# zjhellofss/KuiperLLama

Hardware: NVIDIA H100
Metric: decode_tokens_per_s (higher is better)
Workload: dtype f32

## Files before the change

kuiperllama_b200/csrc/megakernel.cu:

```cuda
#include <cooperative_groups.h>
#include <cuda_bf16.h>
#include <cuda_runtime.h>

#include <cfloat>
#include <cstdint>
#include <algorithm>
#include <cstdio>
#include <cstdlib>
#include <string>
#include <vector>

#include "../../include/kllm_b200.h"
#include "kllm_device.cuh"
#include "kllm_host.h"
#include "kv_fp8.cuh"
#include "megakernel.h"

namespace kllm {
namespace mega {

#define KLLM_MBAR_HINT_NS 20000u
#define KLLM_PHASE_CALL __forceinline__
#define KLLM_STAGE_CALL __noinline__
constexpr int kMaxStages = 16;
constexpr int kConsumerWarps = 8;
constexpr int kConsumerThreads = kConsumerWarps * 32;
constexpr int kSoftmaxThreads = 256;
constexpr int kNormThreads = 128;
constexpr long long kSpinLimit = 120000000000LL;

__device__ __forceinline__ uint32_t smem_u32(const void* p) {
  return static_cast<uint32_t>(__cvta_generic_to_shared(p));
}
__device__ __forceinline__ void mbar_init(uint64_t* b, int count) {
  asm volatile("mbarrier.init.shared::cta.b64 [%0], %1;" ::"r"(smem_u32(b)), "r"(count));
}
__device__ __forceinline__ void mbar_expect_tx(uint64_t* b, uint32_t bytes) {
  asm volatile("mbarrier.arrive.expect_tx.shared::cta.b64 _, [%0], %1;" ::"r"(smem_u32(b)),
               "r"(bytes)
               : "memory");
}
__device__ __forceinline__ void mbar_arrive(uint64_t* b) {
  asm volatile("mbarrier.arrive.shared::cta.b64 _, [%0];" ::"r"(smem_u32(b)) : "memory");
}
__device__ __forceinline__ void mbar_wait(uint64_t* b, uint32_t parity) {
  asm volatile(
      "{\n .reg .pred p;\n WAIT_%=:\n"
      " mbarrier.try_wait.parity.shared::cta.b64 p, [%0], %1, %2;\n"
      " @p bra DONE_%=;\n bra WAIT_%=;\n DONE_%=:\n}" ::"r"(smem_u32(b)),
// ... 130 lines not shown
}

struct Pipe {
  int slot;
  uint32_t parity;
  __device__ __forceinline__ void advance(int stages) {
    if (++slot == stages) {
      slot = 0;
      parity ^= 1u;
    }
  }
};

__shared__ uint64_t g_full_bar[kMaxStages];
__shared__ uint64_t g_empty_bar[kMaxStages];
__shared__ float g_s_warp[kConsumerWarps];
__shared__ float g_s_argv[kConsumerWarps];
__shared__ int g_s_argi[kConsumerWarps];
__shared__ float g_s_bcast;
__shared__ volatile int g_stop;
__shared__ volatile unsigned g_prod_end;
__shared__ Phase g_ph_cons;
__shared__ Phase g_ph_prod;
extern __shared__ __align__(128) unsigned char smem[];
struct Carry {
  Pipe pipe;
  float best_v;
  int best_i;
};

__device__ __forceinline__ void grid_barrier(unsigned* counter, unsigned& target, unsigned grid) {
  consumer_sync();
  target += grid;
  if (threadIdx.x == 0) {
    red_release_add(counter, 1u);
    while (static_cast<int>(ld_acquire_u32(counter) - target) < 0) {
    }
  }
  consumer_sync();
}

struct RowRef {
  int seg;
  int row;
};
__device__ __forceinline__ RowRef resolve_row(const Phase& ph, int unit, int sub) {
// ... 83 lines not shown
    for (int r = 0; r < NR; ++r)
#pragma unroll
      for (int j = 0; j < 4; ++j) wv[r][j] = lds_pack<F>(wp[r] + 32 * PB * j);
#pragma unroll
    for (int j = 0; j < 4; ++j)
#pragma unroll
      for (int r = 0; r < NR; ++r) acc[r][j] = __fadd_rn(dot4_ref(xv[j], wv[r][j]), acc[r][j]);
    xp += 2048;
#pragma unroll
    for (int r = 0; r < NR; ++r) wp[r] += 128 * PB;
  }
  if (full < n_packs) {
#pragma unroll
    for (int j = 0; j < 4; ++j) {
      if (full + 32 * j + lane < n_packs) {
        const float4 xv = lds_f4(xp + 512 * j);
#pragma unroll
        for (int r = 0; r < NR; ++r) acc[r][j] = __fadd_rn(dot4_ref(xv, lds_pack<F>(wp[r] + 32 * PB * j)), acc[r][j]);
      }
    }
  }
}

template <int NR>
__device__ __forceinline__ void accum_w8_g64(const uint32_t (&w)[NR], const uint32_t (&sc)[NR], uint32_t x,
                                             int M, int lane, float (&acc)[NR][4]) {
  const int chunks = M >> 7;
  const bool tail = (chunks << 7) + (lane << 2) < M;
  const int total = chunks + (tail ? 1 : 0);
  if (total == 0) return;
  uint32_t xp = x + lane * 16;
  uint32_t wp[NR], sp[NR];
#pragma unroll
  for (int r = 0; r < NR; ++r) {
    wp[r] = w[r] + lane * 4;
    sp[r] = sc[r] + (lane >> 4) * 4;
  }
  float4 xv = lds_f4(xp);
  uint32_t packed[NR];
  float s[NR];
#pragma unroll
  for (int r = 0; r < NR; ++r) {
    packed[r] = lds_u32(wp[r]);
    s[r] = lds_f32(sp[r]);
  }
#pragma unroll 2
// ... 133 lines not shown
      uint32_t* o1 = reinterpret_cast<uint32_t*>(gb + ((1u + odd) & 3u) * 64);
      uint32_t* o2 = reinterpret_cast<uint32_t*>(gb + ((2u + odd) & 3u) * 64);
#pragma unroll
      for (int j = 0; j < 4; ++j) {
        const float e[4] = {v[j].x, v[j].y, v[j].z, v[j].w};
        uint32_t p0 = 0, p1 = 0, p2 = 0;
#pragma unroll
        for (int b = 0; b < 4; ++b) {
          const int qv = __float2int_rn(e[b] * inv);
          const int a0 = ((qv + 128) & 255) - 128;
          const int q1 = (qv - a0) >> 8;
          const int a1 = ((q1 + 128) & 255) - 128;
          const int a2 = (q1 - a1) >> 8;
          p0 |= static_cast<uint32_t>(a0 & 255) << (8 * b);
          p1 |= static_cast<uint32_t>(a1 & 255) << (8 * b);
          p2 |= static_cast<uint32_t>(a2 & 255) << (8 * b);
        }
        o0[j] = p0, o1[j] = p1, o2[j] = p2;
      }
      if (q == 0) *reinterpret_cast<float*>(gb + ((3u + odd) & 3u) * 64) = step;
    }
  }
  consumer_sync();
}

struct Rows4 {
  uint32_t a[4];
};
template <int NR, WeightFormat F>
__device__ __forceinline__ float4 dot_rows(Rows4 rows, Rows4 scales, uint32_t x, int M, int group_size,
                                           int group_shift, int lane, bool fast = false) {
  float acc[NR][4];
#pragma unroll
  for (int r = 0; r < NR; ++r)
#pragma unroll
    for (int j = 0; j < 4; ++j) acc[r][j] = 0.f;
  float d[4] = {0.f, 0.f, 0.f, 0.f};
  uint32_t w[NR], sc[NR];
#pragma unroll
  for (int r = 0; r < NR; ++r) {
    w[r] = rows.a[r];
    sc[r] = scales.a[r];
  }
  if constexpr (F == WeightFormat::kInt8) {
    if (fast) {
      float a1[NR];
// ... 1148 lines not shown
  return id;
}

template <WeightFormat F, int KV, bool LP, bool PROF>
__device__ __forceinline__ void megakernel_body(const Params& P) {
  uint64_t* full_bar = g_full_bar;
  uint64_t* empty_bar = g_empty_bar;
  Phase& s_phase_cons = g_ph_cons;
  Phase& s_phase_prod = g_ph_prod;

  float* xres = reinterpret_cast<float*>(smem + P.xbuf_bytes);
  unsigned char* stages = smem + P.xbuf_bytes + P.xres_bytes;
  const int S = P.num_stages;
  const int tid = threadIdx.x;
  const int lane = tid & 31;
  const int warp = tid >> 5;
  const bool is_producer = warp == kConsumerWarps;
  const int cta = blockIdx.x;
  const int G = gridDim.x;

  if (tid == 0) {
    g_stop = 0;
    g_prod_end = 0u;
    for (int s = 0; s < S; ++s) {
      mbar_init(&full_bar[s], 1);
      mbar_init(&empty_bar[s], kConsumerWarps);
    }
    asm volatile("fence.mbarrier_init.release.cluster;" ::: "memory");
  }
  __syncthreads();

  Pipe pipe{0, 0u};
  constexpr int wbytes = weight_bytes(F);

  if (is_producer) {
    const uint64_t policy = policy_evict_first();
    const uint64_t policy_kv = policy_evict_last();
    int ppos = P.state->pos;
    unsigned long long* pstamp = nullptr;
    auto claim_slot = [&](uint32_t bytes) -> unsigned char* {
      const long long pw0 = PROF ? clock64() : 0;
      if (mbar_wait_or_stop(&empty_bar[pipe.slot], pipe.parity ^ 1u, &g_stop)) return nullptr;
      if constexpr (PROF) {
        if (pstamp && lane == 0) {
          atomicAdd(pstamp + 11, static_cast<unsigned long long>(clock64() - pw0));
          atomicAdd(pstamp + 12, 1ull);
        }
      }
      if (lane == 0) mbar_expect_tx(&full_bar[pipe.slot], bytes);
      __syncwarp();
      return stages + static_cast<size_t>(pipe.slot) * P.stage_bytes;
    };
    for (int tok = 0; tok < P.n_tokens; ++tok, ++ppos) {
      const int n_run = tok < P.skip_cls_tokens ? P.n_phases - P.n_cls_phases : P.n_phases;
      for (int pi = 0; pi < n_run; ++pi) {
        if constexpr (PROF)
          pstamp = (P.prof != nullptr && tok == P.prof_token)
                       ? P.prof + (static_cast<size_t>(cta) * P.n_phases + pi) * kProfStamps
                       : nullptr;
        {
          const uint32_t* src = reinterpret_cast<const uint32_t*>(P.phases + pi);
          uint32_t* dst = reinterpret_cast<uint32_t*>(&s_phase_prod);
          __syncwarp();
          for (int i = lane; i < static_cast<int>(sizeof(Phase) / 4); i += 32) dst[i] = __ldg(src + i);
          __syncwarp();
        }
        const Phase& ph = s_phase_prod;
        if (ph.kind == kPhaseGather) continue;
        if (ph.kind != kPhaseGemv) {
          const int SP = P.attn_split;
          if (cta >= P.head_num * SP || ppos == 0) continue;
// ... 57 lines not shown
            }
          }
          if (ph.kind != kPhaseAttention) {
            const int dv = hs / SP, T = P.attn_tile_v;
            const float* vbase = P.value_cache + head_block + static_cast<size_t>(split) * P.seq_len * dv;
            const int n_tiles = attn_tiles(ppos, T);
            for (int j = 0; j < n_tiles; ++j) {
              const int t0 = j * T;
              const int nt = min(T, ppos - t0);
              unsigned char* dst = claim_slot(static_cast<uint32_t>(nt) * dv * 4);
              if (dst == nullptr) goto producer_done;
              if (lane == 0)
                bulk_g2s(dst, vbase + static_cast<size_t>(t0) * dv, static_cast<uint32_t>(nt) * dv * 4,
                         &full_bar[pipe.slot], policy_kv);
              pipe.advance(S);
            }
          }
          continue;
        }
        const int u0 = static_cast<int>(static_cast<long long>(cta) * ph.units / G);
        const int u1 = static_cast<int>(static_cast<long long>(cta + 1) * ph.units / G);
        const int rpu = ph.swiglu ? 2 : 1;
        const int row_bytes = ph.in_dim * wbytes;
        if (ph.chunks_per_row == 1) {
          const int ups = ph.rows_per_stage / rpu;
          for (int u = u0; u < u1; u += ups) {
            const int n = min(ups, u1 - u);
            const int nrows = n * rpu;
            unsigned char* dst = claim_slot(static_cast<uint32_t>(nrows) * (row_bytes + ph.scale_row_bytes));
            if (dst == nullptr) goto producer_done;
            const RowRef rr = lane < nrows ? stage_row(ph, u, n, lane) : RowRef{-1, -1};
            const int len = run_length(rr, lane, nrows);
            if (len > 0) {
              const long long e = static_cast<long long>(rr.row) * ph.in_dim;
              const unsigned char* src = static_cast<const unsigned char*>(ph.seg[rr.seg].w) + e * wbytes;
              bulk_g2s(dst + static_cast<size_t>(lane) * row_bytes, src, static_cast<uint32_t>(len) * row_bytes,
                       &full_bar[pipe.slot], policy);
              if (ph.scale_row_bytes) {
                const long long g0 = ph.group_shift >= 0 ? (e >> ph.group_shift) : (e / ph.group_size);
                bulk_g2s(dst + ph.scale_off + static_cast<size_t>(lane) * ph.scale_row_bytes,
                         ph.seg[rr.seg].scales + g0, static_cast<uint32_t>(len) * ph.scale_row_bytes,
                         &full_bar[pipe.slot], policy);
              }
            }
            pipe.advance(S);
          }
        } else {
          for (int u = u0; u < u1; ++u) {
            const RowRef rr = resolve_row(ph, u, 0);
            const unsigned char* src = static_cast<const unsigned char*>(ph.seg[rr.seg].w) +
                                       static_cast<long long>(rr.row) * row_bytes;
            for (int c = 0; c < ph.chunks_per_row; ++c) {
              const int e0 = c * ph.chunk_elems;
              const int ne = min(ph.chunk_elems, ph.in_dim - e0);
              unsigned char* dst = claim_slot(static_cast<uint32_t>(ne) * wbytes);
              if (dst == nullptr) goto producer_done;
              if (lane == 0)
                bulk_g2s(dst, src + static_cast<size_t>(e0) * wbytes, static_cast<uint32_t>(ne) * wbytes,
                         &full_bar[pipe.slot], policy);
              pipe.advance(S);
            }
          }
        }
      }
    }
  producer_done:
    if (lane == 0) g_prod_end = 1u + ((static_cast<unsigned>(pipe.slot) << 1) | pipe.parity);
    return;
  }

  unsigned bar_target = P.barrier_base;
  int token = P.state->token;
  int pos = P.state->pos;
  record_fed(P, pos, token);
  if (static_cast<unsigned>(token) >= static_cast<unsigned>(P.vocab_size)) token = 0;
  int step = P.state->step;
  float4* xres4 = reinterpret_cast<float4*>(xres);
  constexpr int kPhaseWords = static_cast<int>(sizeof(Phase) / 4);
  static_assert(kPhaseWords <= kConsumerThreads, "phase copy: one word per consumer thread");
  uint32_t next_phase_word = tid < kPhaseWords ? __ldg(reinterpret_cast<const uint32_t*>(P.phases) + tid) : 0u;

  for (int tok = 0; tok < P.n_tokens; ++tok) {
    const float* emb_row = P.tok_emb + static_cast<size_t>(token) * P.dim;
    ArgBest best{0.f, -1};
    const float4* e4 = reinterpret_cast<const float4*>(emb_row);
    for (int i = tid; i < (P.dim >> 2); i += kConsumerThreads) xres4[i] = __ldg(e4 + i);

    const bool prof_on = PROF && P.prof != nullptr && tok == P.prof_token && tid == 0;
    auto hand_tag = [&](int hand) {
      return P.hand_base + static_cast<unsigned>(tok * P.hands_per_token + hand) + 1u;
// ... 64 lines not shown
    step += 1;
    if (cta == 0 && tid == 0 && (tok == P.n_tokens - 1 || stop)) {
      P.state->token = token;
      P.state->pos = pos;
      P.state->step = step;
      P.state->next = next;
    }
    if (stop) {
      if (tid == 0) g_stop = 1;
      unsigned end;
      while ((end = g_prod_end) == 0u) {
      }
      const Pipe last{static_cast<int>((end - 1u) >> 1), (end - 1u) & 1u};
      while (pipe.slot != last.slot || pipe.parity != last.parity) {
        mbar_wait(&full_bar[pipe.slot], pipe.parity);
        pipe.advance(S);
      }
      return;
    }
  }
}

template <WeightFormat F, int KV, bool LP, bool PROF>
__global__ void __launch_bounds__(kConsumerThreads + 32, 1) decode_megakernel(const __grid_constant__ Params P) {
  megakernel_body<F, KV, LP, PROF>(P);
}

}

using mega::Params;
using mega::Phase;

namespace {
template <typename K>
const void* fn(K* kernel) {
  return reinterpret_cast<const void*>(kernel);
}
struct Kernels {
  const void *plain, *prof, *lp;
};
template <WeightFormat F, int KV>
Kernels kernels_for() {
  using mega::decode_megakernel;
  const void* prof = nullptr;
  if constexpr (F != WeightFormat::kBf16 && KV == KLLM_KV_F32) prof = fn(decode_megakernel<F, KV, false, true>);
  return Kernels{fn(decode_megakernel<F, KV, false, false>), prof, fn(decode_megakernel<F, KV, true, false>)};
}
template <WeightFormat F>
Kernels kernels_for(int kv) {
  switch (kv) {
    case KLLM_KV_BF16: return kernels_for<F, KLLM_KV_BF16>();
    case KLLM_KV_FP8: return kernels_for<F, KLLM_KV_FP8>();
    default: return kernels_for<F, KLLM_KV_F32>();
  }
}
Kernels kernels_for(WeightFormat f, int kv) {
  switch (f) {
    case WeightFormat::kInt8: return kernels_for<WeightFormat::kInt8>(kv);
    case WeightFormat::kBf16: return kernels_for<WeightFormat::kBf16>(kv);
    default: return kernels_for<WeightFormat::kF32>(kv);
  }
}
constexpr int kThreads = mega::kConsumerThreads + 32;
constexpr int kW16StageBytes = 32 * 1024;
constexpr int kW16FastStageBytes = 24 * 1024;
}

int MegaEngine::init(const DecoderModel& dm, const MegaModel& m, cudaStream_t stream) {
  int dev = 0;
  if (cudaGetDevice(&dev) != cudaSuccess) return KLLM_E_NODEVICE;
  int sms = 0, coop = 0, max_smem = 0;
  KLLM_TRY(cudaDeviceGetAttribute(&sms, cudaDevAttrMultiProcessorCount, dev));
  KLLM_TRY(cudaDeviceGetAttribute(&coop, cudaDevAttrCooperativeLaunch, dev));
  KLLM_TRY(cudaDeviceGetAttribute(&max_smem, cudaDevAttrMaxSharedMemoryPerBlockOptin, dev));
  if (!coop) return KLLM_E_UNSUPPORTED;

  const int dim = dm.dim, hid = dm.hidden_dim, hs = dm.head_size, kvd = dm.kv_dim, q_rows = dm.q_rows;
  const bool int8 = dm.format == WeightFormat::kInt8;
  const bool w16 = dm.format == WeightFormat::kBf16;
  const int wb = weight_bytes(dm.format);
  const int grid = std::min(sms, std::min(dim, hid));
  if (grid < dm.head_num) return KLLM_E_UNSUPPORTED;
  if ((dim & 3) || (hid & 3) || (q_rows & 3) || (hs & 3) || hs > 128) return KLLM_E_UNSUPPORTED;
  if (int8 && ((dim & 15) || (hid & 15) || (q_rows & 15) || (dm.group_size & 3))) return KLLM_E_UNSUPPORTED;
  if (w16 && ((dim & 7) || (hid & 7) || (q_rows & 7))) return KLLM_E_UNSUPPORTED;
  if ((hs * 4) % 16 != 0) return KLLM_E_UNSUPPORTED;
  if (int8) {
    const int dims[3] = {dim, hid, q_rows};
    for (int d : dims)
      if (d % dm.group_size != 0 || ((d / dm.group_size) * 4) % 16 != 0) return KLLM_E_UNSUPPORTED;
  }
  int fast = m.numerics == 1 ? 1 : 0;
  if (const char* e = getenv("KLLM_MODE")) fast = std::string(e) == "fast" ? 1 : 0;
  const int kv = m.kv_cache;
  if (kv != KLLM_KV_F32 && kv != KLLM_KV_BF16 && kv != KLLM_KV_FP8) return KLLM_E_INVALID;
  const int kv_esz = prefill::kv_elem_bytes(kv);
  if (kv != KLLM_KV_F32 && (!fast || m.tp_world > 1 || hs % (64 / kv_esz) != 0)) return KLLM_E_UNSUPPORTED;
  if (kv == KLLM_KV_FP8 && m.kv_scales == nullptr) return KLLM_E_INVALID;
  const Kernels ks = kernels_for(dm.format, kv);

  const int W = m.tp_world > 1 ? m.tp_world : 1;
  if (W != 1 && W != 2 && W != 4 && W != 8) return KLLM_E_UNSUPPORTED;

  const int max_in = std::max(std::max(dim, hid), q_rows);
  int xbuf = max_in * 4;
  const int attn_ws = 2 * hs * 4;
  xbuf = std::max(xbuf, attn_ws);
  const bool small_stages = fast && kv == KLLM_KV_F32 && !w16 && 2 * dim * 4 <= 16 * 1024;
  int stage_bytes = int8 ? 27 * 1024 : w16 ? (fast ? kW16FastStageBytes : kW16StageBytes) : small_stages ? 16 * 1024
                                                                                                : 32 * 1024;
  if (const char* e = getenv("KLLM_STAGE_BYTES")) stage_bytes = atoi(e);
  stage_bytes = (stage_bytes + 127) & ~127;
  const int attn_tile = std::min(stage_bytes / (hs * kv_esz), mega::kConsumerThreads) & ~31;
  if (attn_tile < 32) return KLLM_E_UNSUPPORTED;
  if (fast) {
    if (hs & 15) return KLLM_E_UNSUPPORTED;
    xbuf = std::max(xbuf, (2 * hs + mega::kConsumerWarps * (hs + 2)) * 4);
  }
  xbuf = std::max(xbuf, sampling::kDrawScratchBase + 64 * 8);
  xbuf = std::max(xbuf, sampling::logprob_scratch_bytes(mega::kConsumerThreads));
  xbuf = (xbuf + 127) & ~127;
  const int xres = (dim * 4 + 127) & ~127;
  const int budget = max_smem - xbuf - xres - 3584;
  int stages = budget / stage_bytes;
  if (stages > mega::kMaxStages) stages = mega::kMaxStages;
  if (stages < 2) return KLLM_E_UNSUPPORTED;
  if (dm.seq_len & 3) return KLLM_E_UNSUPPORTED;
  int split = 1;
  while (split * 2 <= 8 && dm.head_num * split * 2 <= grid && (hs / (split * 2)) % 4 == 0 && hs % (split * 2) == 0)
    split *= 2;
  int split_cap = split;
  if (hs < 128) split = 1;
  if (fast) {
    split = 1;
// ... 35 lines not shown
      const int chunk_max = (stage_bytes / wb) & ~511;
      p.chunks_per_row = (p.in_dim + chunk_max - 1) / chunk_max;
      int ce = (p.in_dim + p.chunks_per_row - 1) / p.chunks_per_row;
      ce = (ce + 511) & ~511;
      p.chunk_elems = ce;
      p.chunks_per_row = (p.in_dim + ce - 1) / ce;
      p.rows_per_stage = 1;
      p.scale_off = 0;
    }
    return 0;
  };
  Phase qkv{}, wo{}, ffn{}, w2{}, cls{};
  qkv.in_dim = dim, wo.in_dim = q_rows, ffn.in_dim = dim, ffn.swiglu = 1, w2.in_dim = hid, cls.in_dim = dim;
  for (Phase* p : {&qkv, &wo, &ffn, &w2, &cls})
    if (int rc = plan(*p)) return rc;
  const int V = dm.vocab_size;
  const bool shard = W > 1 && V % W == 0 && m.tp_stride >= V / W;
  const int cls_rows = shard ? V / W : V;

  for (const void* k : {ks.plain, ks.prof, ks.lp})
    if (k != nullptr)
      if (int rc = smem_opt_in(k, smem_bytes)) return rc;
  int occ_lp = 0;
  KLLM_TRY(cudaOccupancyMaxActiveBlocksPerMultiprocessor(&occ_lp, ks.lp, kThreads, smem_bytes));
  if (occ_lp < 1) return KLLM_E_UNSUPPORTED;
  int occ = 0;
  KLLM_TRY(cudaOccupancyMaxActiveBlocksPerMultiprocessor(&occ, ks.plain, kThreads, smem_bytes));
  if (occ < 1) return KLLM_E_UNSUPPORTED;

  const int n_phases = dm.layer_num * ((fast || split == 1) ? 5 : 6) + (shard ? 2 : 1);
  size_t bytes = 0;
  auto part = [&bytes](size_t n) {
    const size_t off = bytes;
    bytes += (n + 255) & ~static_cast<size_t>(255);
    return off;
  };
  using u64 = unsigned long long;
  const size_t hand_off = part(sizeof(u64) * (2 * q_rows + 2 * kvd + hid));
  const size_t scores_off = part(sizeof(u64) * dm.head_num * dm.seq_len);
  const size_t probs_off = part(fast || split == 1 ? 0 : sizeof(float) * dm.head_num * split * dm.seq_len);
  const size_t tagged_off = part(W == 1 ? sizeof(u64) * 2 * dim : 0);
  const size_t phases_off = part(sizeof(Phase) * n_phases);
  const size_t barrier_off = part(128);
  const size_t arg_val_off = part(sizeof(float) * grid), arg_idx_off = part(sizeof(int) * grid);
  const size_t lp_off = part(static_cast<size_t>(grid) * (sizeof(float2) + 8 * sampling::kMaxTopLogprobs));
  KLLM_TRY(cudaMalloc(&scratch_, bytes));
  unsigned char* const s = static_cast<unsigned char*>(scratch_);
  u64 *t_q = reinterpret_cast<u64*>(s + hand_off), *t_k = t_q + q_rows, *t_v = t_k + kvd, *t_attn = t_v + kvd,
      *t_h = t_attn + q_rows;

  std::vector<Phase> ph;
  int hands = 0;
  int exch = 0;
  auto input_is_x = [&](Phase& p) {
    if (exch == 0) return;
    p.tp_in = 1;
    p.exch = exch - 1;
  };

  auto seg = [](const Matrix& w, float* out, int rows, int head_major = 0, unsigned long long* tag_out = nullptr) {
    return mega::Seg{w.w, w.scales, w.bias, out, 0, rows, head_major, tag_out};
  };
  for (int l = 0; l < dm.layer_num; ++l) {
    const LayerWeights& lw = dm.layers[l];
    const size_t layer_off = static_cast<size_t>(l) * dm.seq_len * kvd;
    {
      Phase p = qkv;
      p.kind = mega::kPhaseGemv;
      p.n_seg = 3;
      input_is_x(p);
      p.norm_w = lw.attn_norm;
      p.norm_eps = dm.eps;
      p.seg[0] = seg(lw.q, nullptr, q_rows, 0, t_q);
      p.seg[1] = seg(lw.k, nullptr, kvd, 0, t_k);
      float* vrows = reinterpret_cast<float*>(reinterpret_cast<unsigned char*>(m.value_cache) + layer_off * kv_esz);
      p.seg[2] = seg(lw.v, vrows, kvd, 1, t_v);
      p.layer = l;
      p.units = q_rows + 2 * kvd;
      p.hand_out = hands;
      ph.push_back(p);
    }
    if (fast || split == 1) {
      Phase p{};
      p.kind = fast ? mega::kPhaseAttnFlash : mega::kPhaseAttnFused;
      p.layer = l;
      p.tq = t_q, p.tk = t_k, p.tv = t_v, p.ta = t_attn;
      p.hand_in = hands++;
      p.hand_out = hands;
      ph.push_back(p);
    } else {
      int qkv_hand = 0;
      {
        Phase p{};
        p.kind = mega::kPhaseAttention;
        p.layer = l;
        p.tq = t_q, p.tk = t_k, p.tv = t_v;
        p.hand_in = hands++;
        qkv_hand = p.hand_in;
        p.hand_out = hands;
        ph.push_back(p);
      }
      {
        Phase p{};
        p.kind = mega::kPhaseAttnPV;
        p.layer = l;
        p.hand_in = hands++;
        p.tv = t_v, p.ta = t_attn;
        p.hand_aux = qkv_hand;
        p.hand_out = hands;
        ph.push_back(p);
      }
    }
    {
      Phase p = wo;
      p.kind = mega::kPhaseGemv;
      p.n_seg = 1;
      p.tag_in = t_attn;
      p.hand_in = hands++;
      p.seg[0] = seg(lw.o, nullptr, dim);
      p.units = dim;
      p.tp_out = 1;
      p.exch_out = exch++;
      ph.push_back(p);
    }
    {
      Phase p = ffn;
      p.kind = mega::kPhaseGemv;
      p.n_seg = 2;
      input_is_x(p);
      p.norm_w = lw.ffn_norm;
      p.norm_eps = dm.eps;
      p.seg[0] = seg(lw.w1, nullptr, hid, 0, t_h);
      p.seg[1] = seg(lw.w3, nullptr, hid);
      p.units = hid;
      p.hand_out = hands;
      ph.push_back(p);
    }
    {
      Phase p = w2;
      p.kind = mega::kPhaseGemv;
      p.n_seg = 1;
      p.tag_in = t_h;
      p.hand_in = hands++;
      p.seg[0] = seg(lw.w2, nullptr, dim);
      p.units = dim;
      p.tp_out = 1;
      p.exch_out = exch++;
      ph.push_back(p);
    }
  }
  {
    Phase p = cls;
    p.kind = mega::kPhaseGemv;
    p.n_seg = 1;
    input_is_x(p);
    p.norm_w = dm.final_norm;
    p.norm_eps = dm.eps;
    p.cls = 1;
    if (shard) {
      p.seg[0] = seg(dm.rows_from(dm.cls, static_cast<size_t>(m.tp_rank) * cls_rows, dim), nullptr, cls_rows);
      p.units = cls_rows;
      p.tp_out = 1;
      p.exch_out = exch++;
      ph.push_back(p);
      Phase g{};
      g.kind = mega::kPhaseGather;
      g.cls = 1;
      g.argmax = 1;
      g.units = V;
      g.in_dim = cls_rows;
      g.exch = p.exch_out;
      g.seg[0].out = m.logits;
      ph.push_back(g);
    } else {
      p.seg[0] = seg(dm.cls, m.logits, V);
      p.units = V;
      p.argmax = 1;
      ph.push_back(p);
    }
  }

  KLLM_TRY(cudaMemsetAsync(s, 0, bytes, stream));
  KLLM_TRY(cudaMemcpyAsync(s + phases_off, ph.data(), sizeof(Phase) * n_phases, cudaMemcpyHostToDevice, stream));
  KLLM_TRY(cudaStreamSynchronize(stream));

  Params P{};
  P.phases = reinterpret_cast<const Phase*>(s + phases_off);
  P.n_phases = n_phases;
  P.n_cls_phases = shard ? 2 : 1;
  P.int8_fast = (int8 && fast) ? 1 : 0;
  P.num_stages = stages;
  P.stage_bytes = stage_bytes;
  P.xbuf_bytes = xbuf;
  P.xres_bytes = xres;
  P.attn_tile = attn_tile;
  P.attn_tile_v = attn_tile_v;
  P.attn_split = split;
  P.attn_vsplit = vsplit;
  P.scores = reinterpret_cast<u64*>(s + scores_off);
  P.group_size = dm.group_size;
  P.dim = dm.dim;
  P.vocab_size = dm.vocab_size;
  P.head_num = dm.head_num;
  P.head_size = dm.head_size;
  P.kv_dim = dm.kv_dim;
  P.kv_mul = dm.kv_mul;
  P.seq_len = dm.seq_len;
  P.flavour = dm.flavour;
  P.tok_emb = dm.tok_emb;
  P.score = m.score;
  P.probs = reinterpret_cast<float*>(s + probs_off);
  P.key_cache = m.key_cache;
  P.value_cache = m.value_cache;
  P.sin_cache = m.sin_cache;
  P.cos_cache = m.cos_cache;
  P.state = m.state;
  P.out_tokens = m.out_tokens;
// ... 10 lines not shown
  P.arg_idx = reinterpret_cast<int*>(s + arg_idx_off);
  P.sampling = m.sampling;
  P.logits = m.logits;
  P.hist = m.hist;
  P.penalized = m.penalized;
  P.prof_token = -1;
  for (int i = 0; i < mega::kMaxStopIds; ++i) P.stop_ids[i] = -1;
  P.lp_part = reinterpret_cast<float2*>(s + lp_off);
  P.lp_cand_v = reinterpret_cast<float*>(P.lp_part + grid);
  P.lp_cand_i = reinterpret_cast<int*>(P.lp_cand_v + static_cast<size_t>(grid) * sampling::kMaxTopLogprobs);
  P.lp_rec = m.lp_rec;
  if (kv == KLLM_KV_FP8) {
    const size_t n = static_cast<size_t>(dm.layer_num) * dm.kv_head_num;
    P.kv_scale_k = m.kv_scales, P.kv_scale_v = m.kv_scales + n;
    P.kv_inv_k = m.kv_scales + 2 * n, P.kv_inv_v = m.kv_scales + 3 * n;
  }
  base_ = P;
  stream_ = stream;
  grid_ = grid;
  fast_ = fast;
  cls_rows_ = cls_rows;
  kernel_ = ks.plain, kernel_prof_ = ks.prof, kernel_lp_ = ks.lp;
  smem_bytes_ = smem_bytes;
  ready_ = true;
  return 0;
}

int MegaEngine::destroy() {
  const cudaError_t e = cudaFree(scratch_);
  scratch_ = nullptr;
  ready_ = false;
  return static_cast<int>(e);
}

Params MegaEngine::params(const DrawSettings& cfg, int n_tokens) const {
  Params P = base_;
  P.n_tokens = n_tokens;
  P.penalty = cfg.penalty;
  P.lp_top_n = cfg.lp_top_n;
  P.barrier_base = barrier_base_;
  P.tp_seq_base = tp_seq_base_;
  P.hand_base = hand_base_;
  return P;
}

int MegaEngine::launch(const Params& P) {
  void* args[] = {const_cast<Params*>(&P)};
  const void* k = P.prof != nullptr ? kernel_prof_ : P.lp_top_n >= 0 ? kernel_lp_ : kernel_;
  if (k == nullptr) return KLLM_E_UNSUPPORTED;
  KLLM_TRY(cudaLaunchCooperativeKernel(const_cast<void*>(k), dim3(grid_), dim3(kThreads), args, smem_bytes_, stream_));
  count_launch();
  return 0;
}

void MegaEngine::account(int n_tokens) {
  tp_seq_base_ += static_cast<unsigned>(n_tokens) * static_cast<unsigned>(base_.exch_per_token);
  hand_base_ += static_cast<unsigned>(n_tokens) * static_cast<unsigned>(base_.hands_per_token);
  barrier_base_ += static_cast<unsigned>(n_tokens) * static_cast<unsigned>(grid_);
}

int MegaEngine::run(const DrawSettings& cfg, int n_tokens, const int32_t* teacher_dev, unsigned long long* prof_dev,
                    int prof_token, int skip_cls_tokens, int lp_target) {
  if (!ready_) return KLLM_E_STATE;
  Params P = params(cfg, n_tokens);
  P.teacher = teacher_dev;
  P.prof = prof_dev;
  P.prof_token = prof_token;
  P.skip_cls_tokens = skip_cls_tokens;
  P.lp_target = lp_target;
  if (int rc = launch(P)) return rc;
  account(n_tokens);
  return 0;
}
// ... 14 lines not shown
```

kuiperllama_b200/csrc/megakernel.h:

```cpp
#pragma once
#include <cuda_runtime.h>

#include <cstddef>
#include <cstdint>

#include "decoder_model.h"
#include "sampling.cuh"

namespace kllm {
namespace mega {

enum {
  kPhaseGemv = 0,
  kPhaseAttention = 1 ,
  kPhaseAttnPV = 2 ,
  kPhaseAttnFused = 3 ,
  kPhaseAttnFlash = 4 ,
  kPhaseGather = 5
};
constexpr int kProfStamps = 16;
constexpr int kMaxStopIds = 16;

struct Seg {
  const void* w;
  const float* scales;
  const float* bias;
  float* out;
  long long pos_stride;
  int rows;
  int head_major;
  unsigned long long* tag_out;
};

struct Phase {
  int kind;
  int in_dim;
  int units;
  int n_seg;
  int swiglu;
  int argmax;
  int cls;
  int group_size, group_shift;
  int rows_per_stage;
  int chunks_per_row;
  int chunk_elems;
  int scale_off;
  int scale_row_bytes;
  int layer;
  float norm_eps;
  const float* norm_w;
  int tp_in, tp_out;
  int exch;
  int exch_out;
  const unsigned long long* tag_in;
// ... 5 lines not shown
  int hand_aux;
  Seg seg[3];
};

struct State {
  int32_t token;
  int32_t pos;
  int32_t step;
  int32_t next;
  int32_t teacher;
  int32_t streamed;
  int32_t lp_from;
  int32_t lp_target;
};

struct Params {
  const Phase* phases;
  int n_phases, n_tokens;
  int attn_vsplit;
  int int8_fast;
  int n_cls_phases;
  int skip_cls_tokens;
  int num_stages, stage_bytes, xbuf_bytes;
  int xres_bytes;
  int attn_tile;
  int attn_tile_v;
  unsigned long long* scores;
  int attn_split;
  int group_size;
  int dim, vocab_size, head_num, head_size, kv_dim, kv_mul, seq_len, flavour;
  const float* tok_emb;
  float* score;
  float* probs;
  float* key_cache;
  const float* value_cache;
  const float* sin_cache;
  const float* cos_cache;
  State* state;
  int32_t* out_tokens;
  const int32_t* teacher;
  int max_steps;
  unsigned* barrier;
  unsigned barrier_base;
  unsigned long long* tp_data[8];
  int tp_world, tp_rank, tp_stride, exch_per_token;
  unsigned tp_seq_base;
// ... 46 lines not shown
 public:
  int init(const DecoderModel& dm, const MegaModel& m, cudaStream_t stream);
  int destroy();
  int run(const DrawSettings& cfg, int n_tokens, const int32_t* teacher_dev, unsigned long long* prof_dev = nullptr,
          int prof_token = -1, int skip_cls_tokens = 0, int lp_target = 0);
  int run_until(const DrawSettings& cfg, int n_tokens, const int32_t* stop_ids, int n_stop, int32_t* stream_ids,
                int32_t* stream_count);
  void account(int n_tokens);
  int grid() const { return grid_; }
  int phases() const { return base_.n_phases; }
  int attn_vsplit() const { return base_.attn_vsplit; }
  int fast() const { return fast_; }
  int attn_tile() const { return base_.attn_tile; }
  int attn_split() const { return base_.attn_split; }
  int attn_tile_v() const { return base_.attn_tile_v; }
  int stage_bytes() const { return base_.stage_bytes; }
  int cls_rows() const { return cls_rows_; }

 private:
  mega::Params params(const DrawSettings& cfg, int n_tokens) const;
  int launch(const mega::Params& P);
  mega::Params base_{};
  void* scratch_ = nullptr;
  cudaStream_t stream_ = nullptr;
  unsigned barrier_base_ = 0, tp_seq_base_ = 0, hand_base_ = 0;
  int grid_ = 0;
  int fast_ = 0;
  int cls_rows_ = 0;
  const void* kernel_ = nullptr;
  const void* kernel_prof_ = nullptr;
  const void* kernel_lp_ = nullptr;
  size_t smem_bytes_ = 0;
  bool ready_ = false;
};

}
```

Before: 656.9.

## Stream losslessly exponent-packed f32 weights and expand them in shared memory

At init, each f32 weight row whose exponents span at most 16 values is repacked into 448-byte blocks per 128 elements: three mantissa/sign words plus a 4-bit exponent code per element. Rows that do not fit stay raw, and per-row offset metadata is kept. The producer warp bulk-copies the compressed rows into pipeline stages, and two new decode warps expand each stage back to plain f32 in place before signalling the consumers through a second barrier. The goal is to cut HBM bytes for bandwidth-bound decode by about an eighth. The cost is extra shared-memory traffic, another pipeline hop, more threads per block, and coupling between producer and decoder warps.

Result: slower. 512.1, median of 6 (-22.0%).

```diff
diff --git a/kuiperllama_b200/csrc/megakernel.cu b/kuiperllama_b200/csrc/megakernel.cu
--- a/kuiperllama_b200/csrc/megakernel.cu
+++ b/kuiperllama_b200/csrc/megakernel.cu
@@ -25,6 +25,11 @@
 constexpr int kMaxStages = 16;
 constexpr int kConsumerWarps = 8;
 constexpr int kConsumerThreads = kConsumerWarps * 32;
+constexpr int kDecodeWarps = 2;
+template <WeightFormat F, int KV>
+constexpr int kernel_threads() {
+  return kConsumerThreads + 32 + (F == WeightFormat::kF32 && KV == KLLM_KV_F32 ? 32 * kDecodeWarps : 0);
+}
 constexpr int kSoftmaxThreads = 256;
 constexpr int kNormThreads = 128;
 constexpr long long kSpinLimit = 120000000000LL;
@@ -201,6 +206,10 @@
 __shared__ volatile unsigned g_prod_end;
 __shared__ Phase g_ph_cons;
 __shared__ Phase g_ph_prod;
+__shared__ uint64_t g_land_bar[kMaxStages];
+__shared__ uint32_t g_slot_desc[kMaxStages];
+__shared__ uint32_t g_row_info[kMaxStages * 32];
+__shared__ volatile unsigned g_prod_fills;
 extern __shared__ __align__(128) unsigned char smem[];
 struct Carry {
   Pipe pipe;
@@ -330,6 +339,22 @@
   }
 }
 
+constexpr int kCodeBlockBytes = 448;
+constexpr unsigned long long kCodeOffMask = (1ull << 48) - 1;
+__device__ __forceinline__ uint32_t lds_u16(uint32_t a) {
+  uint32_t v;
+  asm volatile("ld.shared.u16 %0, [%1];" : "=r"(v) : "r"(a));
+  return v;
+}
+__device__ __forceinline__ float4 decode_pack(uint32_t q0, uint32_t q1, uint32_t q2, uint32_t c, uint32_t b0) {
+  constexpr uint32_t kKeep = 0x807fffffu;
+  const uint32_t t0 = ((c & 0xfu) << 23) + b0, t1 = ((c & 0xffu) << 19) + b0, t2 = ((c & 0xfffu) << 15) + b0,
+                 t3 = (c << 11) + b0;
+  const uint32_t v = __byte_perm(__byte_perm(q0 << 1, q1 << 1, 0x0073), q2 << 1, 0x7710);
+  return make_float4(__uint_as_float((q0 & kKeep) | (t0 & ~kKeep)), __uint_as_float((q1 & kKeep) | (t1 & ~kKeep)),
+                     __uint_as_float((q2 & kKeep) | (t2 & ~kKeep)), __uint_as_float((v & kKeep) | (t3 & ~kKeep)));
+}
+
 template <int NR>
 __device__ __forceinline__ void accum_w8_g64(const uint32_t (&w)[NR], const uint32_t (&sc)[NR], uint32_t x,
                                              int M, int lane, float (&acc)[NR][4]) {
@@ -509,6 +534,53 @@
     }
   }
   consumer_sync();
+}
+
+__device__ __forceinline__ void sts_u4(uint32_t a, uint4 v) {
+  asm volatile("st.shared.v4.b32 [%0], {%1,%2,%3,%4};" ::"r"(a), "r"(v.x), "r"(v.y), "r"(v.z), "r"(v.w) : "memory");
+}
+__device__ __forceinline__ void expand_stage(uint32_t base, const uint32_t* info, int nrows, uint32_t rb, int lane) {
+  constexpr int G = 4;
+  for (int j = nrows - 1; j >= 0; --j) {
+    const uint32_t src = base + (info[j] & 0xffffffu), dst = base + static_cast<uint32_t>(j) * rb, b = info[j] >> 24;
+    const int nb = static_cast<int>(rb >> 9);
+    if (b == 0u) {
+      if (src == dst) continue;
+      for (int k = nb - 1; k >= 0; k -= G) {
+        uint4 v[G];
+#pragma unroll
+        for (int g = 0; g < G; ++g) v[g] = lds_u4(src + 512u * max(k - g, 0) + 16u * lane);
+        __syncwarp();
+#pragma unroll
+        for (int g = 0; g < G; ++g)
+          if (k - g >= 0) sts_u4(dst + 512u * (k - g) + 16u * lane, v[g]);
+        __syncwarp();
+      }
+      continue;
+    }
+    const uint32_t b0 = (b - 15u) << 23;
+    for (int k = nb - 1; k >= 0; k -= G) {
+      uint32_t q[G][3], c[G];
+#pragma unroll
+      for (int g = 0; g < G; ++g) {
+        const uint32_t a = src + kCodeBlockBytes * static_cast<uint32_t>(max(k - g, 0));
+        q[g][0] = lds_u32(a + 4u * lane);
+        q[g][1] = lds_u32(a + 128u + 4u * lane);
+        q[g][2] = lds_u32(a + 256u + 4u * lane);
+        c[g] = lds_u16(a + 384u + 2u * lane);
+      }
+      __syncwarp();
+#pragma unroll
+      for (int g = 0; g < G; ++g) {
+        if (k - g >= 0) {
+          const float4 w = decode_pack(q[g][0], q[g][1], q[g][2], c[g], b0);
+          sts_u4(dst + 512u * (k - g) + 16u * lane,
+                 make_uint4(__float_as_uint(w.x), __float_as_uint(w.y), __float_as_uint(w.z), __float_as_uint(w.w)));
+        }
+      }
+      __syncwarp();
+    }
+  }
 }
 
 struct Rows4 {
@@ -1703,9 +1775,11 @@
   if (tid == 0) {
     g_stop = 0;
     g_prod_end = 0u;
+    g_prod_fills = 0u;
     for (int s = 0; s < S; ++s) {
       mbar_init(&full_bar[s], 1);
       mbar_init(&empty_bar[s], kConsumerWarps);
+      mbar_init(&g_land_bar[s], 1);
     }
     asm volatile("fence.mbarrier_init.release.cluster;" ::: "memory");
   }
@@ -1714,12 +1788,40 @@
   Pipe pipe{0, 0u};
   constexpr int wbytes = weight_bytes(F);
 
+  constexpr bool kCodable = F == WeightFormat::kF32 && KV == KLLM_KV_F32;
+  const bool coded_run = kCodable && P.coded != 0;
+
+  if (warp > kConsumerWarps) {
+    if constexpr (kCodable) {
+      const int d = warp - kConsumerWarps - 1;
+      Pipe dp{0, 0u};
+      for (unsigned seq = 0;; ++seq, dp.advance(S)) {
+        if (static_cast<int>(seq % kDecodeWarps) != d) continue;
+        for (;;) {
+          if (mbar_try_wait(&g_land_bar[dp.slot], dp.parity)) break;
+          const unsigned fills = g_prod_fills;
+          if (fills != 0u && seq + 1u >= fills) return;
+        }
+        const uint32_t desc = g_slot_desc[dp.slot];
+        if (desc >> 24)
+          expand_stage(smem_u32(stages + static_cast<size_t>(dp.slot) * P.stage_bytes), g_row_info + dp.slot * 32,
+                       static_cast<int>(desc >> 24), desc & 0xffffffu, lane);
+        asm volatile("fence.proxy.async.shared::cta;" ::: "memory");
+        __syncwarp();
+        if (lane == 0) mbar_arrive(&full_bar[dp.slot]);
+      }
+    }
+    return;
+  }
+
   if (is_producer) {
+    uint64_t* const full_bar = coded_run ? g_land_bar : g_full_bar;
+    unsigned fills = 0;
     const uint64_t policy = policy_evict_first();
     const uint64_t policy_kv = policy_evict_last();
     int ppos = P.state->pos;
     unsigned long long* pstamp = nullptr;
-    auto claim_slot = [&](uint32_t bytes) -> unsigned char* {
+    auto claim_slot = [&](uint32_t bytes, uint32_t desc = 0u, uint32_t info = 0u) -> unsigned char* {
       const long long pw0 = PROF ? clock64() : 0;
       if (mbar_wait_or_stop(&empty_bar[pipe.slot], pipe.parity ^ 1u, &g_stop)) return nullptr;
       if constexpr (PROF) {
@@ -1728,6 +1830,12 @@
           atomicAdd(pstamp + 12, 1ull);
         }
       }
+      if (coded_run) {
+        if (lane == 0) g_slot_desc[pipe.slot] = desc;
+        if (lane < static_cast<int>(desc >> 24)) g_row_info[pipe.slot * 32 + lane] = info;
+        __syncwarp();
+      }
+      ++fills;
       if (lane == 0) mbar_expect_tx(&full_bar[pipe.slot], bytes);
       __syncwarp();
       return stages + static_cast<size_t>(pipe.slot) * P.stage_bytes;
@@ -1831,7 +1939,70 @@
         const int u1 = static_cast<int>(static_cast<long long>(cta + 1) * ph.units / G);
         const int rpu = ph.swiglu ? 2 : 1;
         const int row_bytes = ph.in_dim * wbytes;
-        if (ph.chunks_per_row == 1) {
+        if (coded_run && ph.chunks_per_row == 1) {
+          const int ups = ph.rows_per_stage / rpu;
+          auto load_meta = [&](int u, unsigned long long& a, unsigned long long& b) {
+            const int n = min(ups, u1 - u);
+            a = b = 0;
+            if (u < u1 && lane < n * rpu) {
+              const RowRef rr = stage_row(ph, u, n, lane);
+              const unsigned long long* meta = ph.seg[rr.seg].meta + rr.row;
+              a = __ldg(meta);
+              b = __ldg(meta + 1);
+            }
+          };
+          unsigned long long m0, m1;
+          load_meta(u0, m0, m1);
+          for (int u = u0; u < u1; u += ups) {
+            const int n = min(ups, u1 - u);
+            const int nrows = n * rpu;
+            unsigned long long n0, n1;
+            load_meta(u + ups, n0, n1);
+            const RowRef rr = lane < nrows ? stage_row(ph, u, n, lane) : RowRef{-1, -1};
+            const uint32_t sz = static_cast<uint32_t>((m1 & kCodeOffMask) - (m0 & kCodeOffMask));
+            uint32_t end = sz;
+#pragma unroll
+            for (int d = 1; d < 32; d <<= 1) {
+              const uint32_t t = __shfl_up_sync(kFull, end, d);
+              if (lane >= d) end += t;
+            }
+            const uint32_t start = end - sz;
+            const int len = run_length(rr, lane, nrows);
+            const uint32_t run_end = __shfl_sync(kFull, end, min(lane + max(len, 1) - 1, 31));
+            unsigned char* dst = claim_slot(__shfl_sync(kFull, end, 31),
+                                            static_cast<uint32_t>(row_bytes) | static_cast<uint32_t>(nrows) << 24,
+                                            start | static_cast<uint32_t>(m0 >> 48) << 24);
+            if (dst == nullptr) goto producer_done;
+            if (len > 0)
+              bulk_g2s(dst + start, static_cast<const unsigned char*>(ph.seg[rr.seg].w) + (m0 & kCodeOffMask),
+                       run_end - start, &full_bar[pipe.slot], policy);
+            pipe.advance(S);
+            m0 = n0, m1 = n1;
+          }
+        } else if (coded_run) {
+          auto load_meta = [&](int u) {
+            if (u >= u1) return 0ull;
+            const RowRef rr = resolve_row(ph, u, 0);
+            return __ldg(ph.seg[rr.seg].meta + rr.row);
+          };
+          unsigned long long m0 = load_meta(u0);
+          for (int u = u0; u < u1; ++u) {
+            const unsigned long long next = load_meta(u + 1);
+            const RowRef rr = resolve_row(ph, u, 0);
+            const uint32_t b = static_cast<uint32_t>(m0 >> 48);
+            const unsigned char* src = static_cast<const unsigned char*>(ph.seg[rr.seg].w) + (m0 & kCodeOffMask);
+            for (int c = 0; c < ph.chunks_per_row; ++c) {
+              const int e0 = c * ph.chunk_elems;
+              const int ne = min(ph.chunk_elems, ph.in_dim - e0);
+              const uint32_t at = b ? (e0 >> 7) * kCodeBlockBytes : e0 * 4, bytes = b ? (ne >> 7) * kCodeBlockBytes : ne * 4;
+              unsigned char* dst = claim_slot(bytes, static_cast<uint32_t>(ne) * 4u | 1u << 24, b << 24);
+              if (dst == nullptr) goto producer_done;
+              if (lane == 0) bulk_g2s(dst, src + at, bytes, &full_bar[pipe.slot], policy);
+              pipe.advance(S);
+            }
+            m0 = next;
+          }
+        } else if (ph.chunks_per_row == 1) {
           const int ups = ph.rows_per_stage / rpu;
           for (int u = u0; u < u1; u += ups) {
             const int n = min(ups, u1 - u);
@@ -1874,7 +2045,10 @@
       }
     }
   producer_done:
-    if (lane == 0) g_prod_end = 1u + ((static_cast<unsigned>(pipe.slot) << 1) | pipe.parity);
+    if (lane == 0) {
+      g_prod_end = 1u + ((static_cast<unsigned>(pipe.slot) << 1) | pipe.parity);
+      g_prod_fills = fills + 1u;
+    }
     return;
   }
 
@@ -1985,7 +2159,7 @@
 }
 
 template <WeightFormat F, int KV, bool LP, bool PROF>
-__global__ void __launch_bounds__(kConsumerThreads + 32, 1) decode_megakernel(const __grid_constant__ Params P) {
+__global__ void __launch_bounds__(kernel_threads<F, KV>(), 1) decode_megakernel(const __grid_constant__ Params P) {
   megakernel_body<F, KV, LP, PROF>(P);
 }
 
@@ -2025,9 +2199,103 @@
   }
 }
 constexpr int kThreads = mega::kConsumerThreads + 32;
+constexpr int kCodedThreads = kThreads + 32 * mega::kDecodeWarps;
 constexpr int kW16StageBytes = 32 * 1024;
 constexpr int kW16FastStageBytes = 24 * 1024;
 }
+
+namespace code {
+__global__ void code_size_kernel(const float* w, int rows, int cols, unsigned long long* meta) {
+  const int row = blockIdx.x * (blockDim.x / 32) + threadIdx.x / 32, lane = threadIdx.x & 31;
+  if (row >= rows) return;
+  const uint32_t* r = reinterpret_cast<const uint32_t*>(w) + static_cast<size_t>(row) * cols;
+  uint32_t emax = 0, emin = 255;
+  for (int i = lane; i < cols; i += 32) {
+    const uint32_t e = (__ldg(r + i) >> 23) & 0xffu;
+    emax = max(emax, e);
+    emin = min(emin, e);
+  }
+#pragma unroll
+  for (int off = 16; off > 0; off >>= 1) {
+    emax = max(emax, __shfl_xor_sync(0xffffffffu, emax, off));
+    emin = min(emin, __shfl_xor_sync(0xffffffffu, emin, off));
+  }
+  const bool code = emin >= 1 && emax <= 254 && emin + 15 >= emax && cols % 128 == 0;
+  if (lane == 0)
+    meta[row] = code ? (static_cast<unsigned long long>(cols / 128) * mega::kCodeBlockBytes) |
+                           (static_cast<unsigned long long>(emax) << 48)
+                     : static_cast<unsigned long long>(cols) * 4;
+}
+__global__ void code_pack_kernel(const float* w, int rows, int cols, const unsigned long long* meta,
+                                 unsigned char* out) {
+  const int row = blockIdx.x * (blockDim.x / 32) + threadIdx.x / 32, lane = threadIdx.x & 31;
+  if (row >= rows) return;
+  const unsigned long long m = meta[row];
+  const uint32_t b = static_cast<uint32_t>(m >> 48);
+  const uint4* src = reinterpret_cast<const uint4*>(w + static_cast<size_t>(row) * cols);
+  unsigned char* dst = out + (m & mega::kCodeOffMask);
+  if (b == 0) {
+    for (int i = lane; i < cols / 4; i += 32) reinterpret_cast<uint4*>(dst)[i] = __ldg(src + i);
+    return;
+  }
+  for (int blk = 0; blk < cols / 128; ++blk) {
+    const uint4 f = __ldg(src + blk * 32 + lane);
+    const uint32_t e[4] = {f.x, f.y, f.z, f.w};
+    uint32_t c = 0;
+#pragma unroll
+    for (int i = 0; i < 4; ++i) c |= (((e[i] >> 23) & 0xffu) + 15u - b) << (4 * i);
+    const uint32_t f3 = (f.w & 0x7fffffu) | (f.w >> 31) << 23;
+    unsigned char* blk_at = dst + static_cast<size_t>(blk) * mega::kCodeBlockBytes;
+    uint32_t* q = reinterpret_cast<uint32_t*>(blk_at);
+    q[lane] = (f.x & 0x807fffffu) | (f3 & 0xffu) << 23;
+    q[32 + lane] = (f.y & 0x807fffffu) | ((f3 >> 8) & 0xffu) << 23;
+    q[64 + lane] = (f.z & 0x807fffffu) | ((f3 >> 16) & 0xffu) << 23;
+    reinterpret_cast<uint16_t*>(blk_at + 384)[lane] = static_cast<uint16_t>(c);
+  }
+}
+struct CodeMatrix {
+  const float* w;
+  int rows, cols;
+  size_t meta;
+};
+}
+using code::CodeMatrix;
+
+static int build_code(std::vector<CodeMatrix>& mats, cudaStream_t stream, void** meta_out, void** code_out) {
+  size_t n_meta = 0;
+  for (CodeMatrix& m : mats) {
+    m.meta = n_meta;
+    n_meta += static_cast<size_t>(m.rows) + 1;
+  }
+  KLLM_TRY(cudaMalloc(meta_out, n_meta * sizeof(unsigned long long)));
+  unsigned long long* meta = static_cast<unsigned long long*>(*meta_out);
+  constexpr int kWarps = 8;
+  for (const CodeMatrix& m : mats)
+    code::code_size_kernel<<<(m.rows + kWarps - 1) / kWarps, 32 * kWarps, 0, stream>>>(m.w, m.rows, m.cols, meta + m.meta);
+  KLLM_TRY(cudaGetLastError());
+  std::vector<unsigned long long> h(n_meta);
+  KLLM_TRY(cudaMemcpyAsync(h.data(), meta, n_meta * sizeof(unsigned long long), cudaMemcpyDeviceToHost, stream));
+  KLLM_TRY(cudaStreamSynchronize(stream));
+  unsigned long long off = 0;
+  for (const CodeMatrix& m : mats) {
+    for (int r = 0; r < m.rows; ++r) {
+      unsigned long long& v = h[m.meta + r];
+      const unsigned long long size = v & mega::kCodeOffMask;
+      v = off | (v & ~mega::kCodeOffMask);
+      off += size;
+    }
+    h[m.meta + m.rows] = off;
+  }
+  KLLM_TRY(cudaMalloc(code_out, off));
+  KLLM_TRY(cudaMemcpyAsync(meta, h.data(), n_meta * sizeof(unsigned long long), cudaMemcpyHostToDevice, stream));
+  for (const CodeMatrix& m : mats)
+    code::code_pack_kernel<<<(m.rows + kWarps - 1) / kWarps, 32 * kWarps, 0, stream>>>(
+        m.w, m.rows, m.cols, meta + m.meta, static_cast<unsigned char*>(*code_out));
+  KLLM_TRY(cudaGetLastError());
+  KLLM_TRY(cudaStreamSynchronize(stream));
+  return 0;
+}
+
 
 int MegaEngine::init(const DecoderModel& dm, const MegaModel& m, cudaStream_t stream) {
   int dev = 0;
@@ -2072,7 +2340,10 @@
   const bool small_stages = fast && kv == KLLM_KV_F32 && !w16 && 2 * dim * 4 <= 16 * 1024;
   int stage_bytes = int8 ? 27 * 1024 : w16 ? (fast ? kW16FastStageBytes : kW16StageBytes) : small_stages ? 16 * 1024
                                                                                                 : 32 * 1024;
-  if (const char* e = getenv("KLLM_STAGE_BYTES")) stage_bytes = atoi(e);
+  const char* stage_env = getenv("KLLM_STAGE_BYTES");
+  const bool coded = small_stages && stage_env == nullptr && dm.format == WeightFormat::kF32 && W == 1 &&
+                     dim % 128 == 0 && hid % 128 == 0 && q_rows % 128 == 0;
+  if (stage_env) stage_bytes = atoi(stage_env);
   stage_bytes = (stage_bytes + 127) & ~127;
   const int attn_tile = std::min(stage_bytes / (hs * kv_esz), mega::kConsumerThreads) & ~31;
   if (attn_tile < 32) return KLLM_E_UNSUPPORTED;
@@ -2154,10 +2425,11 @@
     if (k != nullptr)
       if (int rc = smem_opt_in(k, smem_bytes)) return rc;
   int occ_lp = 0;
-  KLLM_TRY(cudaOccupancyMaxActiveBlocksPerMultiprocessor(&occ_lp, ks.lp, kThreads, smem_bytes));
+  const int threads = coded ? kCodedThreads : kThreads;
+  KLLM_TRY(cudaOccupancyMaxActiveBlocksPerMultiprocessor(&occ_lp, ks.lp, threads, smem_bytes));
   if (occ_lp < 1) return KLLM_E_UNSUPPORTED;
   int occ = 0;
-  KLLM_TRY(cudaOccupancyMaxActiveBlocksPerMultiprocessor(&occ, ks.plain, kThreads, smem_bytes));
+  KLLM_TRY(cudaOccupancyMaxActiveBlocksPerMultiprocessor(&occ, ks.plain, threads, smem_bytes));
   if (occ < 1) return KLLM_E_UNSUPPORTED;
 
   const int n_phases = dm.layer_num * ((fast || split == 1) ? 5 : 6) + (shard ? 2 : 1);
@@ -2181,6 +2453,30 @@
   u64 *t_q = reinterpret_cast<u64*>(s + hand_off), *t_k = t_q + q_rows, *t_v = t_k + kvd, *t_attn = t_v + kvd,
       *t_h = t_attn + q_rows;
 
+  std::vector<CodeMatrix> code_mats;
+  if (coded) {
+    auto add = [&](const Matrix& mt, int rows, int cols) {
+      code_mats.push_back({static_cast<const float*>(mt.w), rows, cols, 0});
+    };
+    for (const LayerWeights& lw : dm.layers) {
+      add(lw.q, q_rows, dim), add(lw.k, kvd, dim), add(lw.v, kvd, dim), add(lw.o, dim, q_rows);
+      add(lw.w1, hid, dim), add(lw.w3, hid, dim), add(lw.w2, dim, hid);
+    }
+    add(dm.cls, dm.vocab_size, dim);
+    if (int rc = build_code(code_mats, stream, &code_meta_, &code_)) {
+      destroy();
+      return rc;
+    }
+  }
+  size_t next_code = 0;
+  const u64* code_meta = static_cast<const u64*>(code_meta_);
+  auto code_seg = [&](mega::Seg sg) {
+    if (!coded) return sg;
+    sg.w = code_;
+    sg.meta = code_meta + code_mats[next_code++].meta;
+    return sg;
+  };
+
   std::vector<Phase> ph;
   int hands = 0;
   int exch = 0;
@@ -2191,7 +2487,7 @@
   };
 
   auto seg = [](const Matrix& w, float* out, int rows, int head_major = 0, unsigned long long* tag_out = nullptr) {
-    return mega::Seg{w.w, w.scales, w.bias, out, 0, rows, head_major, tag_out};
+    return mega::Seg{w.w, w.scales, w.bias, out, 0, rows, head_major, tag_out, nullptr};
   };
   for (int l = 0; l < dm.layer_num; ++l) {
     const LayerWeights& lw = dm.layers[l];
@@ -2203,10 +2499,10 @@
       input_is_x(p);
       p.norm_w = lw.attn_norm;
       p.norm_eps = dm.eps;
-      p.seg[0] = seg(lw.q, nullptr, q_rows, 0, t_q);
-      p.seg[1] = seg(lw.k, nullptr, kvd, 0, t_k);
+      p.seg[0] = code_seg(seg(lw.q, nullptr, q_rows, 0, t_q));
+      p.seg[1] = code_seg(seg(lw.k, nullptr, kvd, 0, t_k));
       float* vrows = reinterpret_cast<float*>(reinterpret_cast<unsigned char*>(m.value_cache) + layer_off * kv_esz);
-      p.seg[2] = seg(lw.v, vrows, kvd, 1, t_v);
+      p.seg[2] = code_seg(seg(lw.v, vrows, kvd, 1, t_v));
       p.layer = l;
       p.units = q_rows + 2 * kvd;
       p.hand_out = hands;
@@ -2249,7 +2545,7 @@
       p.n_seg = 1;
       p.tag_in = t_attn;
       p.hand_in = hands++;
-      p.seg[0] = seg(lw.o, nullptr, dim);
+      p.seg[0] = code_seg(seg(lw.o, nullptr, dim));
       p.units = dim;
       p.tp_out = 1;
       p.exch_out = exch++;
@@ -2262,8 +2558,8 @@
       input_is_x(p);
       p.norm_w = lw.ffn_norm;
       p.norm_eps = dm.eps;
-      p.seg[0] = seg(lw.w1, nullptr, hid, 0, t_h);
-      p.seg[1] = seg(lw.w3, nullptr, hid);
+      p.seg[0] = code_seg(seg(lw.w1, nullptr, hid, 0, t_h));
+      p.seg[1] = code_seg(seg(lw.w3, nullptr, hid));
       p.units = hid;
       p.hand_out = hands;
       ph.push_back(p);
@@ -2274,7 +2570,7 @@
       p.n_seg = 1;
       p.tag_in = t_h;
       p.hand_in = hands++;
-      p.seg[0] = seg(lw.w2, nullptr, dim);
+      p.seg[0] = code_seg(seg(lw.w2, nullptr, dim));
       p.units = dim;
       p.tp_out = 1;
       p.exch_out = exch++;
@@ -2305,7 +2601,7 @@
       g.seg[0].out = m.logits;
       ph.push_back(g);
     } else {
-      p.seg[0] = seg(dm.cls, m.logits, V);
+      p.seg[0] = code_seg(seg(dm.cls, m.logits, V));
       p.units = V;
       p.argmax = 1;
       ph.push_back(p);
@@ -2325,6 +2621,7 @@
   P.stage_bytes = stage_bytes;
   P.xbuf_bytes = xbuf;
   P.xres_bytes = xres;
+  P.coded = coded ? 1 : 0;
   P.attn_tile = attn_tile;
   P.attn_tile_v = attn_tile_v;
   P.attn_split = split;
@@ -2381,13 +2678,18 @@
   cls_rows_ = cls_rows;
   kernel_ = ks.plain, kernel_prof_ = ks.prof, kernel_lp_ = ks.lp;
   smem_bytes_ = smem_bytes;
+  threads_ = threads;
   ready_ = true;
   return 0;
 }
 
 int MegaEngine::destroy() {
-  const cudaError_t e = cudaFree(scratch_);
-  scratch_ = nullptr;
+  cudaError_t e = cudaFree(scratch_);
+  for (void* p : {code_meta_, code_}) {
+    const cudaError_t f = cudaFree(p);
+    if (e == cudaSuccess) e = f;
+  }
+  scratch_ = code_meta_ = code_ = nullptr;
   ready_ = false;
   return static_cast<int>(e);
 }
@@ -2407,7 +2709,7 @@
   void* args[] = {const_cast<Params*>(&P)};
   const void* k = P.prof != nullptr ? kernel_prof_ : P.lp_top_n >= 0 ? kernel_lp_ : kernel_;
   if (k == nullptr) return KLLM_E_UNSUPPORTED;
-  KLLM_TRY(cudaLaunchCooperativeKernel(const_cast<void*>(k), dim3(grid_), dim3(kThreads), args, smem_bytes_, stream_));
+  KLLM_TRY(cudaLaunchCooperativeKernel(const_cast<void*>(k), dim3(grid_), dim3(threads_), args, smem_bytes_, stream_));
   count_launch();
   return 0;
 }
diff --git a/kuiperllama_b200/csrc/megakernel.h b/kuiperllama_b200/csrc/megakernel.h
--- a/kuiperllama_b200/csrc/megakernel.h
+++ b/kuiperllama_b200/csrc/megakernel.h
@@ -30,6 +30,7 @@
   int rows;
   int head_major;
   unsigned long long* tag_out;
+  const unsigned long long* meta;
 };
 
 struct Phase {
@@ -81,6 +82,7 @@
   int n_cls_phases;
   int skip_cls_tokens;
   int num_stages, stage_bytes, xbuf_bytes;
+  int coded;
   int xres_bytes;
   int attn_tile;
   int attn_tile_v;
@@ -173,6 +175,8 @@
   int launch(const mega::Params& P);
   mega::Params base_{};
   void* scratch_ = nullptr;
+  void* code_meta_ = nullptr;
+  void* code_ = nullptr;
   cudaStream_t stream_ = nullptr;
   unsigned barrier_base_ = 0, tp_seq_base_ = 0, hand_base_ = 0;
   int grid_ = 0;
@@ -182,6 +186,7 @@
   const void* kernel_prof_ = nullptr;
   const void* kernel_lp_ = nullptr;
   size_t smem_bytes_ = 0;
+  int threads_ = 0;
   bool ready_ = false;
 };
 
```
